# ViTAE-Transformer/SAMRS

Hardware: AMD Instinct MI355X
Metric: images/sec (1024^2, vit_h, 32 boxes/img) SAM box->mask (higher is better)
Workload: dtype f16

## Files before the change

samrs_amd/csrc/encoder_kernels.hip:

```cpp
#include "common.h"
#include "kernels.h"

namespace {

__constant__ float c_mean[3] = {123.675f, 116.28f, 103.53f};
__constant__ float c_std[3] = {58.395f, 57.12f, 57.375f};

template <int PREC>
__global__ void patch_im2col_kernel(const uint8_t* __restrict__ img, uint16_t* __restrict__ A, uint16_t* __restrict__ A_lo,
                                    int n_images, int in_h, int in_w, int grid, int patch) {
    const int P2 = patch * patch;
    const int halves = patch / 8;
    const long total = (long)n_images * grid * grid * patch * halves;
    const long t = (long)blockIdx.x * blockDim.x + threadIdx.x;
    if (t >= total) return;
    const int half = t % halves;
    long u = t / halves;
    const int ky = u % patch; u /= patch;
    const int px = u % grid; u /= grid;
    const int py = u % grid;
    const int im = u / grid;
    const int y = py * patch + ky, x0 = px * patch + half * 8;
    float v[3][8];
#pragma unroll
// ... 421 lines not shown
            const bool real = d0 < HD;
            uint2 o = make_uint2(0u, 0u);
            if (real) {
                o.x = pack2_fast<PREC>(O[dt][4 * g + 0] * inv, O[dt][4 * g + 1] * inv);
                o.y = pack2_fast<PREC>(O[dt][4 * g + 2] * inv, O[dt][4 * g + 3] * inv);
                *reinterpret_cast<uint2*>(orow + d0) = o;
            }
#pragma unroll
            for (int e = 0; e < 4; ++e) {
                const float hv = ET<PREC>::to_float((uint16_t)(((e & 2) ? o.y : o.x) >> (16 * (e & 1))));
                h[4 * g + e] = hv;
                l[4 * g + e] = real ? O[dt][4 * g + e] * inv - hv : 0.f;
                ah = fmaxf(ah, fabsf(hv));
                al = fmaxf(al, fabsf(l[4 * g + e]));
            }
        }
        ah = fmaxf(ah, xhalf_partner(ah));
        al = fmaxf(al, xhalf_partner(al));
        const int bh = mx_scale_byte(ah), bl = mx_scale_byte(al);
        const uint2 ch = make_uint2(fp4_pack8(h, bh), fp4_pack8(h + 8, bh)), cl = make_uint2(fp4_pack8(l, bl), fp4_pack8(l + 8, bl));
        *reinterpret_cast<uint2*>(qh + dt * 16 + 8 * hh) = ch;
        *reinterpret_cast<uint2*>(ql + dt * 16 + 8 * hh) = cl;
        if (hh == 0) {
            const size_t si = mx_scale_index(false, (int)row, head * DT + dt, nst4);
            mx.s_hi[si] = (unsigned char)bh;
            mx.s_lo[si] = (unsigned char)bl;
        }
    }
}

template <int HD>
struct WinCfg {
    static constexpr int WS = 14, N = WS * WS, TK = 2 * WS, NT = N / TK, NP = NT * 32;
    static constexpr int DT = (HD + 31) / 32;
    static constexpr bool ONES = SAMRS_WIN_ONES && DT * 32 > HD;
    __device__ static constexpr int lds_key(int key) { return key + (32 - TK) * (key / TK); }
    static constexpr int VSTR = 228;
    static constexpr int NW = 8, THREADS = NW * 64;
    static constexpr int SSTR = 33;
    static constexpr int K_BYTES = NP * HD * 2;
    static constexpr int VT_BYTES = DT * 32 * VSTR * 2;
    static constexpr int S_BYTES = NW * 32 * SSTR * 4;
    static constexpr int TAB_BYTES = 2 * 32 * HD * 2;
    static constexpr int MAX_D = 1280;
    static constexpr int BIAS_BYTES = 2 * MAX_D * 2;
    static constexpr int LDS_BYTES = K_BYTES + VT_BYTES + S_BYTES + TAB_BYTES + BIAS_BYTES;
};

template <int PREC, int HD, int LO = 0 , int PIPE = 0>
__global__ __launch_bounds__(512) void window_attention_kernel(
    const uint16_t* __restrict__ qkv, const float* __restrict__ qkv_bias, const float* __restrict__ rel_h,
    const float* __restrict__ rel_w, uint16_t* __restrict__ out, int grid, int heads, int n_items,
    uint16_t* __restrict__ out_lo = nullptr , MxOut mx = MxOut(),
    uint32_t lo_heads = 0xffffffffu ) {
    using C = WinCfg<HD>;
    constexpr int KS = HD / 16;
    constexpr bool PL = (PIPE & 1) != 0;
    extern __shared__ __attribute__((aligned(16))) unsigned char smem[];
    uint16_t* Ks = reinterpret_cast<uint16_t*>(smem);
    uint16_t* Vt = reinterpret_cast<uint16_t*>(smem + C::K_BYTES);
    float* Scr = reinterpret_cast<float*>(smem + C::K_BYTES + C::VT_BYTES);
    uint16_t* Tab = reinterpret_cast<uint16_t*>(smem + C::K_BYTES + C::VT_BYTES + C::S_BYTES);
    uint16_t* Bia = Tab + 2 * 32 * HD;

    const int tid = threadIdx.x, lane = tid & 63, wave = tid >> 6;
    const int hh = lane >> 5, ql = lane & 31;
    const int D = heads * HD;
    const int nw = (grid + C::WS - 1) / C::WS;
    const size_t img_rows = (size_t)grid * grid;

    for (int i = tid; i < 2 * 32 * HD; i += C::THREADS) {
        const int t = i / (32 * HD), r = (i / HD) % 32, d = i % HD;
        const float v = r < 2 * C::WS - 1 ? (t ? rel_w : rel_h)[r * HD + d] : 0.f;
        Tab[i] = ET<PREC>::from_float(v);
    }
    for (int i = tid; i < 2 * D; i += C::THREADS) Bia[i] = ET<PREC>::from_float(qkv_bias[D + i]);
    for (int i = tid; i < C::NT * (32 - C::TK) * HD; i += C::THREADS)
        Ks[((i / HD) / (32 - C::TK) * 32 + C::TK + (i / HD) % (32 - C::TK)) * HD + i % HD] = 0;
    for (int i = tid; i < C::DT * 32 * C::VSTR / 2; i += C::THREADS) reinterpret_cast<uint32_t*>(Vt)[i] = 0u;
    if (C::ONES) {
        __syncthreads();
        for (int i = tid; i < C::NP; i += C::THREADS) Vt[HD * C::VSTR + i] = ET<PREC>::from_float(1.0f);
    }

    constexpr int CH = HD / 8;
    constexpr int NKC = C::N * CH, NVI = (C::N / 2) * CH;
    constexpr int PK = (NKC + C::THREADS - 1) / C::THREADS, PV = (NVI + C::THREADS - 1) / C::THREADS;
    const int q = 32 * (wave < C::NT ? wave : 0) + ql;
    const int qc = q < C::N ? q : C::N - 1;
    const int qh = qc / C::WS, qw = qc % C::WS;

    uint4 qf[KS], qfn[PL ? 1 : KS], kreg[PK], v0reg[PV], v1reg[PV];
    auto& qdst = *[&]() { if constexpr (PL) return &qf; else return &qfn; }();
    int n_qoff = -1;
    uint32_t n_pad = 0;
    int n_im = 0, n_head = 0;
#define WIN_TOK(r_, off_, pad_)                                                                                      \
    const int ty_##off_ = y0_ + (r_) / C::WS, tx_##off_ = x0_ + (r_) % C::WS;                                        \
    const bool pad_ = ty_##off_ >= grid || tx_##off_ >= grid;                                                        \
    const int off_ = (min(ty_##off_, grid - 1) * grid + min(tx_##off_, grid - 1)) * (3 * D)
    const uint16_t* n_base = qkv;
    int n_y0 = 0, n_x0 = 0;
#define WIN_HEAD(it_)                                                                                                \
    do {                                                                                                             \
        const int wi_ = (it_) / heads;                                                                               \
        n_head = (it_) % heads;                                                                                      \
        const int win_ = wi_ % (nw * nw);                                                                            \
        n_im = wi_ / (nw * nw);                                                                                      \
        n_y0 = (win_ / nw) * C::WS;                                                                                  \
        n_x0 = (win_ % nw) * C::WS;                                                                                  \
        n_base = qkv + (size_t)n_im * img_rows * (3 * D) + n_head * HD;                                              \
        n_pad = 0u;                                                                                                  \
    } while (0)
#define WIN_LOAD_Q()                                                                                                 \
    do {                                                                                                             \
        const int y0_ = n_y0, x0_ = n_x0;                                                                            \
        WIN_TOK(qc, qo_, qp_);                                                                                       \
        n_qoff = (q < C::N && !qp_) ? qo_ : -1;                                                                      \
        _Pragma("unroll") for (int ks_ = 0; ks_ < KS; ++ks_)                                                         \
            qdst[ks_] = *reinterpret_cast<const uint4*>(n_base + qo_ + 16 * ks_ + 8 * hh);                           \
    } while (0)
    auto slot_field = [](int r, int ch) -> uint32_t { return (uint32_t)(r / C::WS) | ((uint32_t)(r % C::WS) << 4) | ((uint32_t)ch << 8); };
    uint32_t kpk[(PK + 1) / 2], vpk[(PV + 1) / 2];
#pragma unroll
    for (int i = 0; i < (PK + 1) / 2; ++i) kpk[i] = 0u;
#pragma unroll
    for (int i = 0; i < (PV + 1) / 2; ++i) vpk[i] = 0u;
#pragma unroll
    for (int i = 0; i < PK; ++i) {
        const int c = tid + i * C::THREADS;
        if (c < NKC) kpk[i >> 1] |= slot_field(c / CH, c % CH) << (12 * (i & 1));
    }
#pragma unroll
    for (int i = 0; i < PV; ++i) {
        const int c = tid + i * C::THREADS;
        if (c < NVI) vpk[i >> 1] |= slot_field(2 * (c % (C::N / 2)), c / (C::N / 2)) << (12 * (i & 1));
    }
#define WIN_TOK2(dy_, dx_, off_, pad_)                                                                               \
    const int ty_##off_ = y0_ + (dy_), tx_##off_ = x0_ + (dx_);                                                      \
    const bool pad_ = ty_##off_ >= grid || tx_##off_ >= grid;                                                        \
    const int off_ = (min(ty_##off_, grid - 1) * grid + min(tx_##off_, grid - 1)) * (3 * D)
#define WIN_LOAD_K(i_)                                                                                               \
    do {                                                                                                             \
        const int y0_ = n_y0, x0_ = n_x0;                                                                            \
        if (tid + (i_) * C::THREADS < NKC) {                                                                         \
            uint32_t f_ = kpk[(i_) >> 1];                                                                            \
            asm volatile("" : "+v"(f_));           \
            f_ >>= 12 * ((i_) & 1);                                                                                  \
            WIN_TOK2((int)(f_ & 15u), (int)((f_ >> 4) & 15u), ko_, kp_);                                             \
            n_pad |= (uint32_t)kp_ << (i_);                                                                          \
            kreg[i_] = *reinterpret_cast<const uint4*>(n_base + ko_ + D + (int)((f_ >> 8) & 15u) * 8);               \
        }                                                                                                            \
    } while (0)
#define WIN_LOAD_V(i_)                                                                                               \
    do {                                                                                                             \
        const int y0_ = n_y0, x0_ = n_x0;                                                                            \
        if (tid + (i_) * C::THREADS < NVI) {                                                                         \
            uint32_t f_ = vpk[(i_) >> 1];                                                                            \
            asm volatile("" : "+v"(f_));                                                                             \
            f_ >>= 12 * ((i_) & 1);                                                                                  \
            const int dy_ = (int)(f_ & 15u), dx_ = (int)((f_ >> 4) & 15u), ch_ = (int)((f_ >> 8) & 15u);             \
            WIN_TOK2(dy_, dx_, vo0_, vp0_);                                                                          \
            WIN_TOK2(dy_, dx_ + 1, vo1_, vp1_);          \
            n_pad |= ((uint32_t)vp0_ | ((uint32_t)vp1_ << 1)) << (PK + 2 * (i_));                                   \
            v0reg[i_] = *reinterpret_cast<const uint4*>(n_base + vo0_ + 2 * D + ch_ * 8);                            \
            v1reg[i_] = *reinterpret_cast<const uint4*>(n_base + vo1_ + 2 * D + ch_ * 8);                            \
        }                                                                                                            \
    } while (0)
    constexpr int NGK = (PK + 1) / 2, NGRP = 1 + NGK + PV;
    static_assert(NGRP <= C::NT, "issue groups are spread over the key tiles");
#define WIN_GROUP(g_)                                                                                                \
    do {                                                                                                             \
        if ((g_) == 0) { if constexpr (!PL) WIN_LOAD_Q(); }                                                        \
        else if ((g_) <= NGK) {                                                                                      \
            WIN_LOAD_K(2 * ((g_) - 1));                                                                              \
            if (2 * ((g_) - 1) + 1 < PK) WIN_LOAD_K(2 * ((g_) - 1) + 1 < PK ? 2 * ((g_) - 1) + 1 : 0);               \
        } else WIN_LOAD_V((g_) - 1 - NGK < PV ? (g_) - 1 - NGK : 0);                                                 \
    } while (0)
#define WIN_ISSUE(it_)                                                                                               \
    do {                                                                                                             \
        WIN_HEAD(it_);                                                                                               \
        _Pragma("unroll") for (int g_ = 0; g_ < NGRP; ++g_) WIN_GROUP(g_);                                           \
        if constexpr (PL) WIN_LOAD_Q();                                                                              \
    } while (0)

    __syncthreads();
    if constexpr ((PIPE & 2) != 0) {
        if (__builtin_amdgcn_readfirstlane(threadIdx.x) >= 256) __builtin_amdgcn_s_setprio(1);
    }
    int it = blockIdx.x;
#ifdef WIN_TIMING
    unsigned long long wph[6] = {0, 0, 0, 0, 0, 0}, wprev = __builtin_amdgcn_s_memtime();
    const unsigned long long wstart = wprev;
    int n_done = 0;
#define WIN_STAMP(i_) { const unsigned long long tn_ = __builtin_amdgcn_s_memtime(); wph[i_] += tn_ - wprev; wprev = tn_; }
#else
#define WIN_STAMP(i_)
#endif
    if (it < n_items) WIN_ISSUE(it);
    for (; it < n_items; it += gridDim.x) {
        __syncthreads();
        WIN_STAMP(0)
        if (__any(n_pad != 0u)) {
#pragma unroll
            for (int i = 0; i < PK; ++i) {
                const uint4 kb = *reinterpret_cast<const uint4*>(Bia + n_head * HD + ((tid + i * C::THREADS) % CH) * 8);
                kreg[i] = sel4((n_pad >> i) & 1u, kb, kreg[i]);
            }
#pragma unroll
            for (int i = 0; i < PV; ++i) {
                const uint4 vb = *reinterpret_cast<const uint4*>(Bia + D + n_head * HD + ((tid + i * C::THREADS) / (C::N / 2)) % CH * 8);
                v0reg[i] = sel4((n_pad >> (PK + 2 * i)) & 1u, vb, v0reg[i]);
                v1reg[i] = sel4((n_pad >> (PK + 2 * i + 1)) & 1u, vb, v1reg[i]);
            }
        }
#pragma unroll
        for (int i = 0; i < PK; ++i) {
            const int c = tid + i * C::THREADS;
            if (c < NKC) *reinterpret_cast<uint4*>(Ks + C::lds_key(c / CH) * HD + (c % CH) * 8) = kreg[i];
        }
#pragma unroll
        for (int i = 0; i < PV; ++i) {
            const int c = tid + i * C::THREADS;
            if (c < NVI) {
                const int kp = c % (C::N / 2), ch = c / (C::N / 2);
#pragma unroll
                for (int e = 0; e < 8; ++e)
                    *reinterpret_cast<uint32_t*>(Vt + (ch * 8 + e) * C::VSTR + C::lds_key(2 * kp)) = pair_elem(v0reg[i], v1reg[i], e);
            }
        }
        if constexpr (!PL) {
#pragma unroll
            for (int ks = 0; ks < KS; ++ks) qf[ks] = qfn[ks];
        }
        const int qoff = n_qoff;
        const bool qin = qoff >= 0;
        const int im = n_im, head = n_head;
        WIN_STAMP(1)
        __syncthreads();
        WIN_STAMP(2)
        const bool has_next = it + (int)gridDim.x < n_items;
        if (has_next) {
            if (wave >= C::NT) WIN_ISSUE(it + (int)gridDim.x);
            else WIN_HEAD(it + (int)gridDim.x);
        }
        WIN_STAMP(3)
#ifdef WIN_TIMING
        ++n_done;
#endif
        if (wave >= C::NT) continue;

        float* scr = Scr + wave * 32 * C::SSTR + ql * C::SSTR;
        float RH[PL ? 1 : C::WS], BW[16];
        float* rhs = scr;
        {
            const f32x16_t th = tile_times_qT<PREC, HD>(Tab, lane, qf);
            if constexpr (PL) {
                const f32x16_t tw = tile_times_qT<PREC, HD>(Tab + 32 * HD, lane, qf);
#pragma unroll
                for (int r = 0; r < 16; ++r) scr[acc_row(r, hh)] = tw[r];
                wave_lds_sync();
#pragma unroll
                for (int r = 0; r < 16; ++r) {
                    const int c = acc_row(r, hh);
                    BW[r] = c < C::TK ? scr[qw - c % C::WS + C::WS - 1] * LOG2E_F : -INFINITY;
                }
                wave_lds_sync();
#pragma unroll
                for (int r = 0; r < 16; ++r) scr[acc_row(r, hh)] = th[r] * LOG2E_F;
                wave_lds_sync();
                RH[0] = 0.f;
            } else {
#pragma unroll
            for (int r = 0; r < 16; ++r) scr[acc_row(r, hh)] = th[r];
            wave_lds_sync();
#pragma unroll
            for (int j = 0; j < C::WS; ++j) RH[j] = scr[qh - j + C::WS - 1] * LOG2E_F;
            wave_lds_sync();
            const f32x16_t tw = tile_times_qT<PREC, HD>(Tab + 32 * HD, lane, qf);
#pragma unroll
            for (int r = 0; r < 16; ++r) scr[acc_row(r, hh)] = tw[r];
            wave_lds_sync();
#pragma unroll
            for (int r = 0; r < 16; ++r) {
                const int c = acc_row(r, hh);
                BW[r] = c < C::TK ? scr[qw - c % C::WS + C::WS - 1] * LOG2E_F : -INFINITY;
            }
            }
        }

        const float c2 = rsqrtf((float)HD) * LOG2E_F;
        f32x16_t O[C::DT];
#pragma unroll
        for (int dt = 0; dt < C::DT; ++dt)
#pragma unroll
            for (int r = 0; r < 16; ++r) O[dt][r] = 0.f;
        float m_run = -INFINITY, l_run = 0.f;
#ifdef WIN_TIMING
        asm volatile("" :: "v"(RH[0]), "v"(BW[15]));
#endif
        WIN_STAMP(4)

        f32x16_t Sn;
// ... 58 lines not shown
            }
        }
        if constexpr (C::ONES) l_run = ones_row_sum<HD, C::DT>(O, hh);
        else l_run += xhalf_partner(l_run);

#ifdef WIN_TIMING
        asm volatile("" :: "v"(O[0][0]), "v"(O[C::DT - 1][15]), "v"(l_run), "v"(qin), "v"(im), "v"(head));
        WIN_STAMP(5)
        continue;
#endif
        if (qin) {
            const float inv = 1.0f / l_run;
            const size_t orow_i = (size_t)im * img_rows + (size_t)(qoff / (3 * D));
            const size_t obase = orow_i * D + head * HD;
            uint16_t* orow = out + obase;
            if constexpr (LO == 2) store_attention_row_mx<PREC, HD, C::DT>(O, inv, orow, hh, mx, orow_i, head, heads);
            else
#pragma unroll
            for (int dt = 0; dt < C::DT; ++dt)
#pragma unroll
                for (int g = 0; g < 4; ++g) {
                    const int d0 = 32 * dt + 8 * g + 4 * hh;
                    if (d0 < HD) {
                        uint2 o;
                        o.x = pack2_fast<PREC>(O[dt][4 * g + 0] * inv, O[dt][4 * g + 1] * inv);
                        o.y = pack2_fast<PREC>(O[dt][4 * g + 2] * inv, O[dt][4 * g + 3] * inv);
                        *reinterpret_cast<uint2*>(orow + d0) = o;
                        if constexpr (LO == 1) {
                            if ((lo_heads >> (head & 31)) & 1u) {
                                uint2 h, l;
                                split2_pack<PREC>(O[dt][4 * g + 0] * inv, O[dt][4 * g + 1] * inv, h.x, l.x);
                                split2_pack<PREC>(O[dt][4 * g + 2] * inv, O[dt][4 * g + 3] * inv, h.y, l.y);
                                *reinterpret_cast<uint2*>(out_lo + obase + d0) = l;
                            }
                        }
                    }
                }
        }
    }
#ifdef WIN_TIMING
    if (lane == 0) {
        unsigned long long* tp = reinterpret_cast<unsigned long long*>(out) + ((size_t)blockIdx.x * 8 + wave) * 8;
        for (int i = 0; i < 6; ++i) tp[i] = wph[i];
        tp[6] = __builtin_amdgcn_s_memtime() - wstart;
        tp[7] = n_done;
    }
#endif
#undef WIN_ISSUE
#undef WIN_GROUP
#undef WIN_LOAD_V
#undef WIN_LOAD_K
#undef WIN_LOAD_Q
#undef WIN_HEAD
#undef WIN_TOK
#undef WIN_TOK2
}

__device__ __forceinline__ void glds16_sbase(uint32_t voff, const void* sbase, uint32_t m0v) {
    uint32_t keep;
    asm volatile(
        "s_mov_b32 %0, m0\n\t"
        "s_mov_b32 m0, %3\n\t"
        "s_nop 0\n\t"
        "global_load_lds_dwordx4 %1, %2\n\t"
        "s_mov_b32 m0, %0"
        : "=&s"(keep)
        : "v"(voff), "s"(sbase), "s"(m0v)
        : "memory");
}

template <int HD>
__global__ __launch_bounds__(256) void vt_pack_kernel(const uint16_t* __restrict__ qkv, uint16_t* __restrict__ vt, int heads,
                                                      int ntok) {
    __shared__ uint16_t tile[64][HD + 2];
    const int tiles = ntok / 64;
    const int t = blockIdx.x % tiles, P = blockIdx.x / tiles;
    const int head = P % heads, im = P / heads;
    const int D = heads * HD;
    const uint16_t* src = qkv + ((size_t)im * ntok + (size_t)t * 64) * (3 * D) + 2 * D + head * HD;
    constexpr int CH = HD / 8;
    for (int c = threadIdx.x; c < 64 * CH; c += 256) {
        const int r = c / CH, ch = c % CH;
        const uint4 v = *reinterpret_cast<const uint4*>(src + (size_t)r * (3 * D) + ch * 8);
        uint32_t* p = reinterpret_cast<uint32_t*>(&tile[r][ch * 8]);
        p[0] = v.x; p[1] = v.y; p[2] = v.z; p[3] = v.w;
    }
    __syncthreads();
    uint16_t* dst = vt + (size_t)P * HD * ntok + (size_t)t * 64;
    for (int c = threadIdx.x; c < HD * 8; c += 256) {
        const int d = c / 8, c8 = c % 8, k0 = 16 * (c8 >> 1) + 4 * (c8 & 1);
        uint4 o;
        o.x = tile[k0 + 0][d] | ((uint32_t)tile[k0 + 1][d] << 16);
        o.y = tile[k0 + 2][d] | ((uint32_t)tile[k0 + 3][d] << 16);
        o.z = tile[k0 + 8][d] | ((uint32_t)tile[k0 + 9][d] << 16);
        o.w = tile[k0 + 10][d] | ((uint32_t)tile[k0 + 11][d] << 16);
        *reinterpret_cast<uint4*>(dst + (size_t)d * ntok + c8 * 8) = o;
    }
}

template <int HD, int NW = 4>
struct GlbCfg {
    static constexpr int G = 64, KT = 64;
    static constexpr int DT = (HD + 31) / 32;
    static constexpr int VSTR = KT + 8;
    static constexpr int KSTR = HD + 8;
    static constexpr int K_BYTES = KT * KSTR * 2;
    static constexpr int VT_BYTES = DT * 32 * VSTR * 2;
// ... 506 lines not shown
        mean += d * (1.0f / (g + 1));
        m2 += gq + d * d * (160.0f * g / (g + 1));
    }
    const float rstd = 1.0f / sqrtf(m2 * (1.0f / 1280.0f) + eps);
    rowstat[row] = make_float2(rstd, -rstd * mean);
}

hipError_t launch_ln_rowstat(const float* stats, float* rowstat, int rows, float eps, hipStream_t s) {
    if (rows < 1 || !stats || !rowstat) return hipErrorInvalidValue;
    ln_rowstat_kernel<<<(rows + 255) / 256, 256, 0, s>>>(reinterpret_cast<const float4*>(stats), reinterpret_cast<float2*>(rowstat), rows, eps);
    return hipGetLastError();
}

hipError_t launch_rowstats_convert(int prec, const float* X, void* Xh, float* stats, int rows, int D, hipStream_t s) {
    if (D != 1280 || rows < 1) return hipErrorInvalidValue;
    const int blocks = (rows + 3) / 4;
    if (prec == PREC_BF16) rowstats_convert_kernel<PREC_BF16><<<blocks, 256, 0, s>>>(X, (uint16_t*)Xh, reinterpret_cast<float2*>(stats), rows);
    else rowstats_convert_kernel<PREC_F16><<<blocks, 256, 0, s>>>(X, (uint16_t*)Xh, reinterpret_cast<float2*>(stats), rows);
    return hipGetLastError();
}

hipError_t launch_layernorm(int prec, const float* X, const float* gamma, const float* beta, float eps,
                            void* out_et, float* out_f32, int rows_out, int D, int window_mode, int grid,
                            int window, hipStream_t s, void* out_lo, void* mx_q_hi, void* mx_q_lo, void* mx_s_hi, void* mx_s_lo, int ld_out,
                            const int* oc_idx, int n_oc) {
    if (D % 4 || D > LN_MAXV * 256) return hipErrorInvalidValue;
    if (ld_out == 0) ld_out = D;
    if (ld_out < D || ld_out % 4 || (ld_out != D && out_lo)) return hipErrorInvalidValue;
    if (n_oc < 0 || n_oc > 32 || (n_oc && (!oc_idx || !out_et || window_mode || ld_out < D + 64))) return hipErrorInvalidValue;
    MxOut mx;
    if (mx_q_hi) {
        if (!mx_q_lo || !mx_s_hi || !mx_s_lo || !out_et || window_mode || D % MXK) return hipErrorInvalidValue;
        mx.q_hi = (unsigned char*)mx_q_hi; mx.q_lo = (unsigned char*)mx_q_lo; mx.s_hi = (unsigned char*)mx_s_hi; mx.s_lo = (unsigned char*)mx_s_lo;
    }
    const int blocks = (rows_out + 3) / 4;
    if (prec == PREC_BF16)
        layernorm_kernel<PREC_BF16><<<blocks, 256, 0, s>>>(X, gamma, beta, eps, (uint16_t*)out_et, out_f32, rows_out, D, window_mode, grid, window, (uint16_t*)out_lo, mx, ld_out, oc_idx, n_oc);
    else
        layernorm_kernel<PREC_F16><<<blocks, 256, 0, s>>>(X, gamma, beta, eps, (uint16_t*)out_et, out_f32, rows_out, D, window_mode, grid, window, (uint16_t*)out_lo, mx, ld_out, oc_idx, n_oc);
    return hipGetLastError();
}

template <int PREC, int HD, int LO = 0>
static hipError_t launch_win(const void* qkv, const float* qb, const float* rh, const float* rw, void* out, int n_images,
                             int grid, int heads, hipStream_t s, void* out_lo = nullptr, MxOut mx = MxOut(), uint32_t lo_heads = 0xffffffffu) {
    using C = WinCfg<HD>;
#ifdef SAMRS_EXPERIMENTS
    static const int pipe = [] { const char* v = getenv("SAMRS_WIN_PIPE"); return v ? atoi(v) & 3 : 0; }();
    auto k = pipe == 3 ? window_attention_kernel<PREC, HD, LO, 3> : pipe == 2 ? window_attention_kernel<PREC, HD, LO, 2>
           : pipe == 1 ? window_attention_kernel<PREC, HD, LO, 1> : window_attention_kernel<PREC, HD, LO, 0>;
#else
    auto k = window_attention_kernel<PREC, HD, LO, 0>;
#endif
    HIP_CHECK_RET(set_lds(k, C::LDS_BYTES));
    if (heads * HD > C::MAX_D) return hipErrorInvalidValue;
    const int nw = (grid + C::WS - 1) / C::WS;
    const int n_items = n_images * nw * nw * heads;
    static const int n_cu = [] {
        int dev = 0, n = 256;
        if (hipGetDevice(&dev) == hipSuccess) (void)hipDeviceGetAttribute(&n, hipDeviceAttributeMultiprocessorCount, dev);
        return n > 0 ? n : 256;
    }();
    dim3 g(n_items < n_cu ? n_items : n_cu), b(C::THREADS);
    k<<<g, b, C::LDS_BYTES, s>>>((const uint16_t*)qkv, qb, rh, rw, (uint16_t*)out, grid, heads, n_items, (uint16_t*)out_lo, mx, lo_heads);
    return hipGetLastError();
}

hipError_t launch_window_attention(int prec, const void* qkv, const float* qkv_bias, const float* rel_h, const float* rel_w, void* out,
                                   int n_images, int grid, int window, int heads, int head_dim, hipStream_t s, void* out_lo,
                                   void* mx_q_hi, void* mx_q_lo, void* mx_s_hi, void* mx_s_lo, uint32_t lo_heads) {
    if (window != 14) return hipErrorInvalidValue;
    if (heads > 32) lo_heads = 0xffffffffu;
    MxOut mx;
    if (mx_q_hi) {
        if (!mx_q_lo || !mx_s_hi || !mx_s_lo || (heads * ((head_dim + 31) / 32) * 32) % MXK) return hipErrorInvalidValue;
        mx.q_hi = (unsigned char*)mx_q_hi; mx.q_lo = (unsigned char*)mx_q_lo; mx.s_hi = (unsigned char*)mx_s_hi; mx.s_lo = (unsigned char*)mx_s_lo;
    }
#define WIN_CALL(P, H)                                                                                                          \
    return mx_q_hi ? launch_win<P, H, 2>(qkv, qkv_bias, rel_h, rel_w, out, n_images, grid, heads, s, nullptr, mx)               \
         : out_lo ? launch_win<P, H, 1>(qkv, qkv_bias, rel_h, rel_w, out, n_images, grid, heads, s, out_lo, MxOut(), lo_heads)  \
                  : launch_win<P, H, 0>(qkv, qkv_bias, rel_h, rel_w, out, n_images, grid, heads, s)
    if (prec == PREC_BF16) {
        if (head_dim == 64) WIN_CALL(PREC_BF16, 64);
        if (head_dim == 80) WIN_CALL(PREC_BF16, 80);
    } else if (prec == PREC_F16) {
        if (head_dim == 64) WIN_CALL(PREC_F16, 64);
        if (head_dim == 80) WIN_CALL(PREC_F16, 80);
    }
#undef WIN_CALL
    return hipErrorInvalidValue;
}

static int g_glb_waves = [] { const char* v = getenv("SAMRS_GLB_WAVES"); return (v && atoi(v) == 4) ? 4 : 8; }();

template <int PREC, int HD, int NW, int LO = 0>
static hipError_t launch_glb_nw(const void* qkv, const float* rh, const float* rw, void* out, int n_images,
                                int heads, void* vt_ws, hipStream_t s, void* out_lo = nullptr, MxOut mx = MxOut()) {
    using C = GlbCfg<HD, NW>;
    constexpr int NTOK = C::G * C::G;
#ifdef SAMRS_EXPERIMENTS
    static const bool pipe = [] { const char* v = getenv("SAMRS_GLB_PIPE"); return v ? atoi(v) != 0 : false; }();
    auto k = pipe ? global_attention_kernel<PREC, HD, NW, LO, 1> : global_attention_kernel<PREC, HD, NW, LO, 0>;
#else
    auto k = global_attention_kernel<PREC, HD, NW, LO, 0>;
#endif
    HIP_CHECK_RET(set_lds(k, C::LDS_BYTES));
    dim3 g((NTOK / (32 * NW)) * heads * n_images), b(64 * NW);
    k<<<g, b, C::LDS_BYTES, s>>>((const uint16_t*)qkv, (const uint16_t*)vt_ws, rh, rw, (uint16_t*)out, heads, (uint16_t*)out_lo, mx);
    return hipGetLastError();
}

template <int PREC, int HD>
static hipError_t launch_glb(const void* qkv, const float* rh, const float* rw, void* out, int n_images,
                             int heads, void* vt_ws, hipStream_t s, void* out_lo, MxOut mx) {
    constexpr int NTOK = GlbCfg<HD>::G * GlbCfg<HD>::G;
    vt_pack_kernel<HD><<<n_images * heads * (NTOK / 64), 256, 0, s>>>((const uint16_t*)qkv, (uint16_t*)vt_ws, heads, NTOK);
    HIP_CHECK_RET(hipGetLastError());
// ... 59 lines not shown
```

samrs_amd/csrc/upscaler_fused.hip:

```cpp
#include "common.h"
#include "kernels.h"

namespace {

constexpr int UF_THREADS = 512;
constexpr int UF_ROWS = 16;

struct UFArgs {
    const uint16_t *keys, *keys_lo;
    const uint16_t *w1, *w1_lo;
    const float* b1;
    const float* ln;
    const uint16_t *w2, *w2_lo;
    const float* b2;
    const float* hyper;
    float* low;
    int tokens, grid, n_mask_tokens, sel0, n_tiles;
};

template <int PREC, int NSEL, bool SPLIT>
__global__ __launch_bounds__(UF_THREADS) void upscaler_fused_kernel(UFArgs a) {
    extern __shared__ __attribute__((aligned(16))) unsigned char uf_lds[];
    unsigned char* At = uf_lds;
    uint4* W2f = reinterpret_cast<uint4*>(uf_lds + 16384);
    float* Part = reinterpret_cast<float*>(uf_lds + 16384 + 32768);
    float* Out = Part + 4 * 2 * 16 * 64;
    float* cst = Out + 3 * 4 * 64;
    const int tid = threadIdx.x, lane = tid & 63;
    const int wave = __builtin_amdgcn_readfirstlane(tid >> 6);
    const int s1 = wave >> 1, p = wave & 1;
    const int fr = lane & 15, fq = lane >> 4;

    uint4 wf1[4][4], wl1[SPLIT ? 4 : 1][4];
#pragma unroll
    for (int i = 0; i < 4; ++i)
#pragma unroll
        for (int ks = 0; ks < 4; ++ks) {
            const size_t o = (size_t)(s1 * 64 + i * 16 + fr) * 256 + (4 * p + ks) * 32 + fq * 8;
            wf1[i][ks] = *reinterpret_cast<const uint4*>(a.w1 + o);
            if constexpr (SPLIT) wl1[i][ks] = *reinterpret_cast<const uint4*>(a.w1_lo + o);
        }
    for (int idx = tid; idx < 8 * 2 * 64; idx += UF_THREADS) {
        const int i2 = idx >> 7, ks2 = (idx >> 6) & 1, l = idx & 63, r_ = l & 15, q_ = l >> 4;
        const size_t o0 = (size_t)(i2 * 16 + r_) * 64 + 16 * (2 * ks2) + 4 * q_, o1 = o0 + 16;
        const uint2 x0 = *reinterpret_cast<const uint2*>(a.w2 + o0), x1 = *reinterpret_cast<const uint2*>(a.w2 + o1);
        W2f[idx] = make_uint4(x0.x, x0.y, x1.x, x1.y);
        if constexpr (SPLIT) {
            const uint2 y0 = *reinterpret_cast<const uint2*>(a.w2_lo + o0), y1 = *reinterpret_cast<const uint2*>(a.w2_lo + o1);
            W2f[8 * 2 * 64 + idx] = make_uint4(y0.x, y0.y, y1.x, y1.y);
        }
    }
    for (int i = tid; i < 512; i += UF_THREADS)
        cst[i] = i < 256 ? a.b1[i] : (i < 384 ? a.ln[i - 256] : a.b2[i - 384]);

    const int tiles_per_prompt = a.tokens / UF_ROWS;
    const int S = 4 * a.grid;
    const int prow = tid >> 5, pch = tid & 31;
    int tile = blockIdx.x;
    uint4 nh = make_uint4(0u, 0u, 0u, 0u), nl = nh;
    if (tile < a.n_tiles) {
        const size_t o = ((size_t)tile * UF_ROWS + prow) * 256 + pch * 8;
        nh = *reinterpret_cast<const uint4*>(a.keys + o);
        if constexpr (SPLIT) nl = *reinterpret_cast<const uint4*>(a.keys_lo + o);
    }
    for (; tile < a.n_tiles; tile += gridDim.x) {
        const int b = tile / tiles_per_prompt, t0 = (tile - b * tiles_per_prompt) * UF_ROWS;
        *reinterpret_cast<uint4*>(At + ((prow * 32 + (pch ^ prow)) << 4)) = nh;
        if constexpr (SPLIT) *reinterpret_cast<uint4*>(At + 8192 + ((prow * 32 + (pch ^ prow)) << 4)) = nl;
        __syncthreads();
        {
            const int nt = tile + (int)gridDim.x;
            if (nt < a.n_tiles) {
                const size_t o = ((size_t)nt * UF_ROWS + prow) * 256 + pch * 8;
                nh = *reinterpret_cast<const uint4*>(a.keys + o);
                if constexpr (SPLIT) nl = *reinterpret_cast<const uint4*>(a.keys_lo + o);
            }
        }
        float hy[NSEL][8];
#pragma unroll
        for (int c = 0; c < NSEL; ++c) {
            const float* h = a.hyper + ((size_t)b * a.n_mask_tokens + a.sel0 + c) * 32;
#pragma unroll
            for (int half = 0; half < 2; ++half) {
                const float4 t = *reinterpret_cast<const float4*>(h + half * 16 + 4 * fq);
                hy[c][half * 4 + 0] = t.x; hy[c][half * 4 + 1] = t.y; hy[c][half * 4 + 2] = t.z; hy[c][half * 4 + 3] = t.w;
            }
        }
        f32x4_t acc[4];
#pragma unroll
        for (int i = 0; i < 4; ++i) acc[i] = f32x4_t{0.f, 0.f, 0.f, 0.f};
#pragma unroll
        for (int ks = 0; ks < 4; ++ks) {
            const int pos = (fr * 32 + (((4 * p + ks) * 4 + fq) ^ fr)) << 4;
            const uint4 af = *reinterpret_cast<const uint4*>(At + pos);
            if constexpr (SPLIT) {
                const uint4 al = *reinterpret_cast<const uint4*>(At + 8192 + pos);
#pragma unroll
                for (int i = 0; i < 4; ++i) acc[i] = ET<PREC>::mfma16(wf1[i][ks], al, acc[i]);
#pragma unroll
                for (int i = 0; i < 4; ++i) acc[i] = ET<PREC>::mfma16(wl1[i][ks], af, acc[i]);
            }
#pragma unroll
            for (int i = 0; i < 4; ++i) acc[i] = ET<PREC>::mfma16(wf1[i][ks], af, acc[i]);
        }
        float* mine = Part + ((s1 * 2 + p) * 16) * 64 + lane;
#pragma unroll
        for (int i = 0; i < 4; ++i)
#pragma unroll
            for (int r = 0; r < 4; ++r) mine[(i * 4 + r) * 64] = acc[i][r];
        __syncthreads();
        float v[4][4];
        float s = 0.f;
        {
            const float* p0 = Part + ((s1 * 2 + 0) * 16) * 64 + lane;
            const float* p1 = Part + ((s1 * 2 + 1) * 16) * 64 + lane;
#pragma unroll
            for (int i = 0; i < 4; ++i) {
                const float4 bb = *reinterpret_cast<const float4*>(cst + s1 * 64 + i * 16 + 4 * fq);
                const float bv[4] = {bb.x, bb.y, bb.z, bb.w};
#pragma unroll
                for (int r = 0; r < 4; ++r) {
                    v[i][r] = (p0[(i * 4 + r) * 64] + p1[(i * 4 + r) * 64]) + bv[r];
                    s += v[i][r];
                }
            }
        }
        s += __shfl_xor(s, 16, 64);
        s += __shfl_xor(s, 32, 64);
        const float mean = s * (1.0f / 64.0f);
        float q = 0.f;
#pragma unroll
        for (int i = 0; i < 4; ++i)
#pragma unroll
            for (int r = 0; r < 4; ++r) { v[i][r] -= mean; q += v[i][r] * v[i][r]; }
        q += __shfl_xor(q, 16, 64);
        q += __shfl_xor(q, 32, 64);
        const float rstd = 1.0f / sqrtf(q * (1.0f / 64.0f) + 1e-6f);
        uint4 bh[2], bl[2];
#pragma unroll
        for (int ks2 = 0; ks2 < 2; ++ks2) {
            uint32_t hh[4], ll[4];
#pragma unroll
            for (int k = 0; k < 2; ++k) {
                const int i = 2 * ks2 + k;
                const float4 gm = *reinterpret_cast<const float4*>(cst + 256 + i * 16 + 4 * fq);
                const float4 bt = *reinterpret_cast<const float4*>(cst + 320 + i * 16 + 4 * fq);
                const float2_t g01 = gelu_erf2(float2_t{v[i][0] * rstd * gm.x + bt.x, v[i][1] * rstd * gm.y + bt.y});
                const float2_t g23 = gelu_erf2(float2_t{v[i][2] * rstd * gm.z + bt.z, v[i][3] * rstd * gm.w + bt.w});
                split2_pack<PREC>(g01.x, g01.y, hh[2 * k], ll[2 * k]);
                split2_pack<PREC>(g23.x, g23.y, hh[2 * k + 1], ll[2 * k + 1]);
            }
            bh[ks2] = make_uint4(hh[0], hh[1], hh[2], hh[3]);
            bl[ks2] = make_uint4(ll[0], ll[1], ll[2], ll[3]);
        }
        float part[NSEL][2];
#pragma unroll
        for (int c = 0; c < NSEL; ++c) part[c][0] = part[c][1] = 0.f;
#pragma unroll
        for (int il = 0; il < 4; ++il) {
            const int i2 = 4 * p + il;
            f32x4_t d = {0.f, 0.f, 0.f, 0.f};
            const uint4 w0 = W2f[(i2 * 2 + 0) * 64 + lane], w1 = W2f[(i2 * 2 + 1) * 64 + lane];
            if constexpr (SPLIT) {
                const uint4 x0 = W2f[8 * 2 * 64 + (i2 * 2 + 0) * 64 + lane], x1 = W2f[8 * 2 * 64 + (i2 * 2 + 1) * 64 + lane];
                d = ET<PREC>::mfma16(w0, bl[0], d);
                d = ET<PREC>::mfma16(w1, bl[1], d);
                d = ET<PREC>::mfma16(x0, bh[0], d);
                d = ET<PREC>::mfma16(x1, bh[1], d);
            }
            d = ET<PREC>::mfma16(w0, bh[0], d);
            d = ET<PREC>::mfma16(w1, bh[1], d);
            const float4 bb = *reinterpret_cast<const float4*>(cst + 384 + i2 * 16 + 4 * fq);
            const float2_t g01 = gelu_erf2(float2_t{d[0] + bb.x, d[1] + bb.y});
            const float2_t g23 = gelu_erf2(float2_t{d[2] + bb.z, d[3] + bb.w});
#pragma unroll
            for (int c = 0; c < NSEL; ++c) {
                const float* h = hy[c] + (il & 1) * 4;
                part[c][il >> 1] += h[0] * g01.x + h[1] * g01.y + h[2] * g23.x + h[3] * g23.y;
            }
        }
#pragma unroll
        for (int c = 0; c < NSEL; ++c)
#pragma unroll
            for (int sl = 0; sl < 2; ++sl) {
                float x = part[c][sl];
                x += __shfl_xor(x, 16, 64);
                x += __shfl_xor(x, 32, 64);
                if (fq == sl) {
                    const int s2 = 2 * p + sl;
                    Out[(c * 4 + 2 * (s1 >> 1) + (s2 >> 1)) * 64 + 4 * fr + 2 * (s1 & 1) + (s2 & 1)] = x;
                }
            }
        __syncthreads();
        for (int idx = tid; idx < NSEL * 256; idx += UF_THREADS) {
            const int c = idx >> 8, yl = (idx >> 6) & 3, xl = idx & 63;
            const int y = t0 / a.grid, x0 = t0 - y * a.grid;
            a.low[(((size_t)b * NSEL + c) * S + 4 * y + yl) * S + 4 * x0 + xl] = Out[(c * 4 + yl) * 64 + xl];
        }
    }
}

constexpr int UF_LDS = 16384 + 32768 + 32768 + 3 * 4 * 64 * 4 + 512 * 4;

}

hipError_t launch_upscaler_fused(int prec, const void* keys, const void* keys_lo, const void* w1, const void* w1_lo, const float* b1,
                                 const float* ln, const void* w2, const void* w2_lo, const float* b2, const float* hyper, float* low,
                                 int n, int grid, int n_mask_tokens, int sel0, int n_sel, hipStream_t s) {
    const bool split = keys_lo && w1_lo && w2_lo;
    if ((keys_lo || w1_lo || w2_lo) && !split) return hipErrorInvalidValue;
    if (n < 1 || grid % UF_ROWS || (n_sel != 1 && n_sel != 3)) return hipErrorInvalidValue;
    static const int n_cu = [] {
        int dev = 0, c = 256;
        if (hipGetDevice(&dev) == hipSuccess) (void)hipDeviceGetAttribute(&c, hipDeviceAttributeMultiprocessorCount, dev);
        return c > 0 ? c : 256;
    }();
    UFArgs a;
    a.keys = (const uint16_t*)keys; a.keys_lo = (const uint16_t*)keys_lo;
    a.w1 = (const uint16_t*)w1; a.w1_lo = (const uint16_t*)w1_lo; a.b1 = b1; a.ln = ln;
    a.w2 = (const uint16_t*)w2; a.w2_lo = (const uint16_t*)w2_lo; a.b2 = b2; a.hyper = hyper; a.low = low;
    a.tokens = grid * grid; a.grid = grid; a.n_mask_tokens = n_mask_tokens; a.sel0 = sel0;
    a.n_tiles = n * (a.tokens / UF_ROWS);
    const int blocks = a.n_tiles < n_cu ? a.n_tiles : n_cu;
#define UF_LAUNCH(P, NS, SP)                                                                                                 \
    do {                                                                                                                     \
        auto k = upscaler_fused_kernel<P, NS, SP>;                                                                           \
        HIP_CHECK_RET(hipFuncSetAttribute(reinterpret_cast<const void*>(k), hipFuncAttributeMaxDynamicSharedMemorySize, UF_LDS)); \
        k<<<blocks, UF_THREADS, UF_LDS, s>>>(a);                                                                             \
    } while (0)
#define UF_SEL(P, SP) do { if (n_sel == 1) UF_LAUNCH(P, 1, SP); else UF_LAUNCH(P, 3, SP); } while (0)
    if (prec == PREC_BF16) { if (split) UF_SEL(PREC_BF16, true); else UF_SEL(PREC_BF16, false); }
    else if (prec == PREC_F16) { if (split) UF_SEL(PREC_F16, true); else UF_SEL(PREC_F16, false); }
    else return hipErrorInvalidValue;
#undef UF_SEL
#undef UF_LAUNCH
    return hipGetLastError();
}
```

Before: 147.5.

## Skip padded query strips in window attention; widen upscaler tile to two groups

The window attention kernel now computes the real query count of each edge window and lets waves whose 32-query strip is entirely padding skip the attention math, with a fast reciprocal-multiply replacing the division for row/column. Separately, the fused upscaler processes two 16-token groups per tile, which halves tile-loop iterations and reuses the register-resident weights across more rows at the cost of roughly doubled LDS. Both paths are on by default and can be switched off through environment variables.

```diff
diff --git a/samrs_amd/csrc/encoder_kernels.hip b/samrs_amd/csrc/encoder_kernels.hip
--- a/samrs_amd/csrc/encoder_kernels.hip
+++ b/samrs_amd/csrc/encoder_kernels.hip
@@ -497,7 +497,8 @@
     const uint16_t* __restrict__ qkv, const float* __restrict__ qkv_bias, const float* __restrict__ rel_h,
     const float* __restrict__ rel_w, uint16_t* __restrict__ out, int grid, int heads, int n_items,
     uint16_t* __restrict__ out_lo = nullptr , MxOut mx = MxOut(),
-    uint32_t lo_heads = 0xffffffffu ) {
+    uint32_t lo_heads = 0xffffffffu ,
+    int dense = 1 ) {
     using C = WinCfg<HD>;
     constexpr int KS = HD / 16;
     constexpr bool PL = (PIPE & 1) != 0;
@@ -509,6 +510,7 @@
     uint16_t* Bia = Tab + 2 * 32 * HD;
 
     const int tid = threadIdx.x, lane = tid & 63, wave = tid >> 6;
+    const int wave_u = __builtin_amdgcn_readfirstlane(wave);
     const int hh = lane >> 5, ql = lane & 31;
     const int D = heads * HD;
     const int nw = (grid + C::WS - 1) / C::WS;
@@ -532,20 +534,20 @@
     constexpr int NKC = C::N * CH, NVI = (C::N / 2) * CH;
     constexpr int PK = (NKC + C::THREADS - 1) / C::THREADS, PV = (NVI + C::THREADS - 1) / C::THREADS;
     const int q = 32 * (wave < C::NT ? wave : 0) + ql;
-    const int qc = q < C::N ? q : C::N - 1;
-    const int qh = qc / C::WS, qw = qc % C::WS;
+    auto slot_row = [](int q_, int vw_) -> int { return (int)(((uint32_t)q_ * ((65536u + (uint32_t)vw_ - 1u) / (uint32_t)vw_)) >> 16); };
 
     uint4 qf[KS], qfn[PL ? 1 : KS], kreg[PK], v0reg[PV], v1reg[PV];
     auto& qdst = *[&]() { if constexpr (PL) return &qf; else return &qfn; }();
     int n_qoff = -1;
     uint32_t n_pad = 0;
     int n_im = 0, n_head = 0;
-#define WIN_TOK(r_, off_, pad_)                                                                                      \
-    const int ty_##off_ = y0_ + (r_) / C::WS, tx_##off_ = x0_ + (r_) % C::WS;                                        \
+#define WIN_TOK2(dy_, dx_, off_, pad_)                                                                               \
+    const int ty_##off_ = y0_ + (dy_), tx_##off_ = x0_ + (dx_);                                                      \
     const bool pad_ = ty_##off_ >= grid || tx_##off_ >= grid;                                                        \
     const int off_ = (min(ty_##off_, grid - 1) * grid + min(tx_##off_, grid - 1)) * (3 * D)
     const uint16_t* n_base = qkv;
     int n_y0 = 0, n_x0 = 0;
+    int n_vw = C::WS, n_nq = C::N;
 #define WIN_HEAD(it_)                                                                                                \
     do {                                                                                                             \
         const int wi_ = (it_) / heads;                                                                               \
@@ -556,12 +558,15 @@
         n_x0 = (win_ % nw) * C::WS;                                                                                  \
         n_base = qkv + (size_t)n_im * img_rows * (3 * D) + n_head * HD;                                              \
         n_pad = 0u;                                                                                                  \
+        n_vw = dense ? min(C::WS, grid - n_x0) : C::WS;                                                              \
+        n_nq = dense ? min(C::WS, grid - n_y0) * n_vw : C::N;                                                        \
     } while (0)
 #define WIN_LOAD_Q()                                                                                                 \
     do {                                                                                                             \
         const int y0_ = n_y0, x0_ = n_x0;                                                                            \
-        WIN_TOK(qc, qo_, qp_);                                                                                       \
-        n_qoff = (q < C::N && !qp_) ? qo_ : -1;                                                                      \
+        const int qc_ = min(q, n_nq - 1), qh_ = slot_row(qc_, n_vw);                                                 \
+        WIN_TOK2(qh_, qc_ - qh_ * n_vw, qo_, qp_);                                                                   \
+        n_qoff = (q < n_nq && !qp_) ? qo_ : -1;                                                                      \
         _Pragma("unroll") for (int ks_ = 0; ks_ < KS; ++ks_)                                                         \
             qdst[ks_] = *reinterpret_cast<const uint4*>(n_base + qo_ + 16 * ks_ + 8 * hh);                           \
     } while (0)
@@ -581,10 +586,6 @@
         const int c = tid + i * C::THREADS;
         if (c < NVI) vpk[i >> 1] |= slot_field(2 * (c % (C::N / 2)), c / (C::N / 2)) << (12 * (i & 1));
     }
-#define WIN_TOK2(dy_, dx_, off_, pad_)                                                                               \
-    const int ty_##off_ = y0_ + (dy_), tx_##off_ = x0_ + (dx_);                                                      \
-    const bool pad_ = ty_##off_ >= grid || tx_##off_ >= grid;                                                        \
-    const int off_ = (min(ty_##off_, grid - 1) * grid + min(tx_##off_, grid - 1)) * (3 * D)
 #define WIN_LOAD_K(i_)                                                                                               \
     do {                                                                                                             \
         const int y0_ = n_y0, x0_ = n_x0;                                                                            \
@@ -681,19 +682,21 @@
         const int qoff = n_qoff;
         const bool qin = qoff >= 0;
         const int im = n_im, head = n_head;
+        const int n_strips = (n_nq + 31) >> 5;
+        const int qc = min(q, n_nq - 1), qh = slot_row(qc, n_vw), qw = qc - qh * n_vw;
         WIN_STAMP(1)
         __syncthreads();
         WIN_STAMP(2)
         const bool has_next = it + (int)gridDim.x < n_items;
         if (has_next) {
-            if (wave >= C::NT) WIN_ISSUE(it + (int)gridDim.x);
+            if (wave_u >= n_strips) WIN_ISSUE(it + (int)gridDim.x);
             else WIN_HEAD(it + (int)gridDim.x);
         }
         WIN_STAMP(3)
 #ifdef WIN_TIMING
         ++n_done;
 #endif
-        if (wave >= C::NT) continue;
+        if (wave_u >= n_strips) continue;
 
         float* scr = Scr + wave * 32 * C::SSTR + ql * C::SSTR;
         float RH[PL ? 1 : C::WS], BW[16];
@@ -858,7 +861,6 @@
 #undef WIN_LOAD_K
 #undef WIN_LOAD_Q
 #undef WIN_HEAD
-#undef WIN_TOK
 #undef WIN_TOK2
 }
 
@@ -1471,6 +1473,7 @@
 #else
     auto k = window_attention_kernel<PREC, HD, LO, 0>;
 #endif
+    static const int dense = [] { const char* v = getenv("SAMRS_WIN_DENSE"); return (v && atoi(v) == 0) ? 0 : 1; }();
     HIP_CHECK_RET(set_lds(k, C::LDS_BYTES));
     if (heads * HD > C::MAX_D) return hipErrorInvalidValue;
     const int nw = (grid + C::WS - 1) / C::WS;
@@ -1481,7 +1484,8 @@
         return n > 0 ? n : 256;
     }();
     dim3 g(n_items < n_cu ? n_items : n_cu), b(C::THREADS);
-    k<<<g, b, C::LDS_BYTES, s>>>((const uint16_t*)qkv, qb, rh, rw, (uint16_t*)out, grid, heads, n_items, (uint16_t*)out_lo, mx, lo_heads);
+    k<<<g, b, C::LDS_BYTES, s>>>((const uint16_t*)qkv, qb, rh, rw, (uint16_t*)out, grid, heads, n_items, (uint16_t*)out_lo, mx, lo_heads,
+                                 dense);
     return hipGetLastError();
 }
 
diff --git a/samrs_amd/csrc/upscaler_fused.hip b/samrs_amd/csrc/upscaler_fused.hip
--- a/samrs_amd/csrc/upscaler_fused.hip
+++ b/samrs_amd/csrc/upscaler_fused.hip
@@ -1,10 +1,12 @@
+#include <cstdlib>
+
 #include "common.h"
 #include "kernels.h"
 
 namespace {
 
 constexpr int UF_THREADS = 512;
-constexpr int UF_ROWS = 16;
+constexpr int UF_GROUP = 16;
 
 struct UFArgs {
     const uint16_t *keys, *keys_lo;
@@ -18,14 +20,16 @@
     int tokens, grid, n_mask_tokens, sel0, n_tiles;
 };
 
-template <int PREC, int NSEL, bool SPLIT>
+template <int PREC, int NSEL, bool SPLIT, int NH >
 __global__ __launch_bounds__(UF_THREADS) void upscaler_fused_kernel(UFArgs a) {
     extern __shared__ __attribute__((aligned(16))) unsigned char uf_lds[];
+    constexpr int ROWS = NH * UF_GROUP;
+    constexpr int AT_LO = ROWS * 512;
     unsigned char* At = uf_lds;
-    uint4* W2f = reinterpret_cast<uint4*>(uf_lds + 16384);
-    float* Part = reinterpret_cast<float*>(uf_lds + 16384 + 32768);
-    float* Out = Part + 4 * 2 * 16 * 64;
-    float* cst = Out + 3 * 4 * 64;
+    uint4* W2f = reinterpret_cast<uint4*>(uf_lds + 2 * AT_LO);
+    float* Part = reinterpret_cast<float*>(uf_lds + 2 * AT_LO + 32768);
+    float* Out = Part + 4 * 2 * NH * 16 * 64;
+    float* cst = Out + 3 * NH * 4 * 64;
     const int tid = threadIdx.x, lane = tid & 63;
     const int wave = __builtin_amdgcn_readfirstlane(tid >> 6);
     const int s1 = wave >> 1, p = wave & 1;
@@ -53,27 +57,39 @@
     for (int i = tid; i < 512; i += UF_THREADS)
         cst[i] = i < 256 ? a.b1[i] : (i < 384 ? a.ln[i - 256] : a.b2[i - 384]);
 
-    const int tiles_per_prompt = a.tokens / UF_ROWS;
+    const int tiles_per_prompt = a.tokens / ROWS;
     const int S = 4 * a.grid;
     const int prow = tid >> 5, pch = tid & 31;
     int tile = blockIdx.x;
-    uint4 nh = make_uint4(0u, 0u, 0u, 0u), nl = nh;
+    uint4 nh[NH], nl[NH];
+#pragma unroll
+    for (int h = 0; h < NH; ++h) nh[h] = nl[h] = make_uint4(0u, 0u, 0u, 0u);
     if (tile < a.n_tiles) {
-        const size_t o = ((size_t)tile * UF_ROWS + prow) * 256 + pch * 8;
-        nh = *reinterpret_cast<const uint4*>(a.keys + o);
-        if constexpr (SPLIT) nl = *reinterpret_cast<const uint4*>(a.keys_lo + o);
+#pragma unroll
+        for (int h = 0; h < NH; ++h) {
+            const size_t o = ((size_t)tile * ROWS + h * UF_GROUP + prow) * 256 + pch * 8;
+            nh[h] = *reinterpret_cast<const uint4*>(a.keys + o);
+            if constexpr (SPLIT) nl[h] = *reinterpret_cast<const uint4*>(a.keys_lo + o);
+        }
     }
     for (; tile < a.n_tiles; tile += gridDim.x) {
-        const int b = tile / tiles_per_prompt, t0 = (tile - b * tiles_per_prompt) * UF_ROWS;
-        *reinterpret_cast<uint4*>(At + ((prow * 32 + (pch ^ prow)) << 4)) = nh;
-        if constexpr (SPLIT) *reinterpret_cast<uint4*>(At + 8192 + ((prow * 32 + (pch ^ prow)) << 4)) = nl;
+        const int b = tile / tiles_per_prompt, t0 = (tile - b * tiles_per_prompt) * ROWS;
+#pragma unroll
+        for (int h = 0; h < NH; ++h) {
+            const int pos = (((h * UF_GROUP + prow) * 32 + (pch ^ prow)) << 4);
+            *reinterpret_cast<uint4*>(At + pos) = nh[h];
+            if constexpr (SPLIT) *reinterpret_cast<uint4*>(At + AT_LO + pos) = nl[h];
+        }
         __syncthreads();
         {
             const int nt = tile + (int)gridDim.x;
             if (nt < a.n_tiles) {
-                const size_t o = ((size_t)nt * UF_ROWS + prow) * 256 + pch * 8;
-                nh = *reinterpret_cast<const uint4*>(a.keys + o);
-                if constexpr (SPLIT) nl = *reinterpret_cast<const uint4*>(a.keys_lo + o);
+#pragma unroll
+                for (int h = 0; h < NH; ++h) {
+                    const size_t o = ((size_t)nt * ROWS + h * UF_GROUP + prow) * 256 + pch * 8;
+                    nh[h] = *reinterpret_cast<const uint4*>(a.keys + o);
+                    if constexpr (SPLIT) nl[h] = *reinterpret_cast<const uint4*>(a.keys_lo + o);
+                }
             }
         }
         float hy[NSEL][8];
@@ -86,34 +102,38 @@
                 hy[c][half * 4 + 0] = t.x; hy[c][half * 4 + 1] = t.y; hy[c][half * 4 + 2] = t.z; hy[c][half * 4 + 3] = t.w;
             }
         }
-        f32x4_t acc[4];
-#pragma unroll
-        for (int i = 0; i < 4; ++i) acc[i] = f32x4_t{0.f, 0.f, 0.f, 0.f};
-#pragma unroll
-        for (int ks = 0; ks < 4; ++ks) {
-            const int pos = (fr * 32 + (((4 * p + ks) * 4 + fq) ^ fr)) << 4;
-            const uint4 af = *reinterpret_cast<const uint4*>(At + pos);
-            if constexpr (SPLIT) {
-                const uint4 al = *reinterpret_cast<const uint4*>(At + 8192 + pos);
-#pragma unroll
-                for (int i = 0; i < 4; ++i) acc[i] = ET<PREC>::mfma16(wf1[i][ks], al, acc[i]);
-#pragma unroll
-                for (int i = 0; i < 4; ++i) acc[i] = ET<PREC>::mfma16(wl1[i][ks], af, acc[i]);
-            }
-#pragma unroll
-            for (int i = 0; i < 4; ++i) acc[i] = ET<PREC>::mfma16(wf1[i][ks], af, acc[i]);
-        }
-        float* mine = Part + ((s1 * 2 + p) * 16) * 64 + lane;
-#pragma unroll
-        for (int i = 0; i < 4; ++i)
-#pragma unroll
-            for (int r = 0; r < 4; ++r) mine[(i * 4 + r) * 64] = acc[i][r];
+#pragma unroll
+        for (int h = 0; h < NH; ++h) {
+            f32x4_t acc[4];
+#pragma unroll
+            for (int i = 0; i < 4; ++i) acc[i] = f32x4_t{0.f, 0.f, 0.f, 0.f};
+#pragma unroll
+            for (int ks = 0; ks < 4; ++ks) {
+                const int pos = ((h * UF_GROUP + fr) * 32 + (((4 * p + ks) * 4 + fq) ^ fr)) << 4;
+                const uint4 af = *reinterpret_cast<const uint4*>(At + pos);
+                if constexpr (SPLIT) {
+                    const uint4 al = *reinterpret_cast<const uint4*>(At + AT_LO + pos);
+#pragma unroll
+                    for (int i = 0; i < 4; ++i) acc[i] = ET<PREC>::mfma16(wf1[i][ks], al, acc[i]);
+#pragma unroll
+                    for (int i = 0; i < 4; ++i) acc[i] = ET<PREC>::mfma16(wl1[i][ks], af, acc[i]);
+                }
+#pragma unroll
+                for (int i = 0; i < 4; ++i) acc[i] = ET<PREC>::mfma16(wf1[i][ks], af, acc[i]);
+            }
+            float* mine = Part + (((s1 * 2 + p) * NH + h) * 16) * 64 + lane;
+#pragma unroll
+            for (int i = 0; i < 4; ++i)
+#pragma unroll
+                for (int r = 0; r < 4; ++r) mine[(i * 4 + r) * 64] = acc[i][r];
+        }
         __syncthreads();
+        const int hg = NH == 2 ? p : 0;
         float v[4][4];
         float s = 0.f;
         {
-            const float* p0 = Part + ((s1 * 2 + 0) * 16) * 64 + lane;
-            const float* p1 = Part + ((s1 * 2 + 1) * 16) * 64 + lane;
+            const float* p0 = Part + (((s1 * 2 + 0) * NH + hg) * 16) * 64 + lane;
+            const float* p1 = Part + (((s1 * 2 + 1) * NH + hg) * 16) * 64 + lane;
 #pragma unroll
             for (int i = 0; i < 4; ++i) {
                 const float4 bb = *reinterpret_cast<const float4*>(cst + s1 * 64 + i * 16 + 4 * fq);
@@ -153,12 +173,16 @@
             bh[ks2] = make_uint4(hh[0], hh[1], hh[2], hh[3]);
             bl[ks2] = make_uint4(ll[0], ll[1], ll[2], ll[3]);
         }
-        float part[NSEL][2];
-#pragma unroll
-        for (int c = 0; c < NSEL; ++c) part[c][0] = part[c][1] = 0.f;
-#pragma unroll
-        for (int il = 0; il < 4; ++il) {
-            const int i2 = 4 * p + il;
+        constexpr int NS2 = 2 * NH;
+        const int s2_0 = NH == 2 ? 0 : 2 * p;
+        float part[NSEL];
+#pragma unroll
+        for (int il = 0; il < 2 * NS2; ++il) {
+            if ((il & 1) == 0) {
+#pragma unroll
+                for (int c = 0; c < NSEL; ++c) part[c] = 0.f;
+            }
+            const int i2 = 2 * s2_0 + il;
             f32x4_t d = {0.f, 0.f, 0.f, 0.f};
             const uint4 w0 = W2f[(i2 * 2 + 0) * 64 + lane], w1 = W2f[(i2 * 2 + 1) * 64 + lane];
             if constexpr (SPLIT) {
@@ -176,31 +200,30 @@
 #pragma unroll
             for (int c = 0; c < NSEL; ++c) {
                 const float* h = hy[c] + (il & 1) * 4;
-                part[c][il >> 1] += h[0] * g01.x + h[1] * g01.y + h[2] * g23.x + h[3] * g23.y;
-            }
-        }
-#pragma unroll
-        for (int c = 0; c < NSEL; ++c)
-#pragma unroll
-            for (int sl = 0; sl < 2; ++sl) {
-                float x = part[c][sl];
-                x += __shfl_xor(x, 16, 64);
-                x += __shfl_xor(x, 32, 64);
-                if (fq == sl) {
-                    const int s2 = 2 * p + sl;
-                    Out[(c * 4 + 2 * (s1 >> 1) + (s2 >> 1)) * 64 + 4 * fr + 2 * (s1 & 1) + (s2 & 1)] = x;
-                }
-            }
+                part[c] += h[0] * g01.x + h[1] * g01.y + h[2] * g23.x + h[3] * g23.y;
+            }
+            if (il & 1) {
+                const int sl = il >> 1, s2 = s2_0 + sl;
+#pragma unroll
+                for (int c = 0; c < NSEL; ++c) {
+                    float x = part[c];
+                    x += __shfl_xor(x, 16, 64);
+                    x += __shfl_xor(x, 32, 64);
+                    if (fq == sl) Out[((c * NH + hg) * 4 + 2 * (s1 >> 1) + (s2 >> 1)) * 64 + 4 * fr + 2 * (s1 & 1) + (s2 & 1)] = x;
+                }
+            }
+        }
         __syncthreads();
-        for (int idx = tid; idx < NSEL * 256; idx += UF_THREADS) {
-            const int c = idx >> 8, yl = (idx >> 6) & 3, xl = idx & 63;
-            const int y = t0 / a.grid, x0 = t0 - y * a.grid;
-            a.low[(((size_t)b * NSEL + c) * S + 4 * y + yl) * S + 4 * x0 + xl] = Out[(c * 4 + yl) * 64 + xl];
+        for (int idx = tid; idx < NSEL * NH * 256; idx += UF_THREADS) {
+            const int ch = idx >> 8, c = ch / NH, tg = t0 + (ch % NH) * UF_GROUP, yl = (idx >> 6) & 3, xl = idx & 63;
+            const int y = tg / a.grid, x0 = tg - y * a.grid;
+            a.low[(((size_t)b * NSEL + c) * S + 4 * y + yl) * S + 4 * x0 + xl] = Out[(ch * 4 + yl) * 64 + xl];
         }
     }
 }
 
-constexpr int UF_LDS = 16384 + 32768 + 32768 + 3 * 4 * 64 * 4 + 512 * 4;
+constexpr int uf_lds_bytes(int nh) { return nh * 16384 + 32768 + nh * 32768 + 3 * nh * 4 * 64 * 4 + 512 * 4; }
+static_assert(uf_lds_bytes(2) <= 160 * 1024, "the 32-token tile must fit the CU's LDS");
 
 }
 
@@ -209,7 +232,8 @@
                                  int n, int grid, int n_mask_tokens, int sel0, int n_sel, hipStream_t s) {
     const bool split = keys_lo && w1_lo && w2_lo;
     if ((keys_lo || w1_lo || w2_lo) && !split) return hipErrorInvalidValue;
-    if (n < 1 || grid % UF_ROWS || (n_sel != 1 && n_sel != 3)) return hipErrorInvalidValue;
+    if (n < 1 || grid % UF_GROUP || (n_sel != 1 && n_sel != 3)) return hipErrorInvalidValue;
+    static const int n_groups = [] { const char* v = getenv("SAMRS_UPSCALER_TILE"); return (v && atoi(v) == 16) ? 1 : 2; }();
     static const int n_cu = [] {
         int dev = 0, c = 256;
         if (hipGetDevice(&dev) == hipSuccess) (void)hipDeviceGetAttribute(&c, hipDeviceAttributeMultiprocessorCount, dev);
@@ -220,13 +244,14 @@
     a.w1 = (const uint16_t*)w1; a.w1_lo = (const uint16_t*)w1_lo; a.b1 = b1; a.ln = ln;
     a.w2 = (const uint16_t*)w2; a.w2_lo = (const uint16_t*)w2_lo; a.b2 = b2; a.hyper = hyper; a.low = low;
     a.tokens = grid * grid; a.grid = grid; a.n_mask_tokens = n_mask_tokens; a.sel0 = sel0;
-    a.n_tiles = n * (a.tokens / UF_ROWS);
+    a.n_tiles = n * (a.tokens / (n_groups * UF_GROUP));
     const int blocks = a.n_tiles < n_cu ? a.n_tiles : n_cu;
 #define UF_LAUNCH(P, NS, SP)                                                                                                 \
     do {                                                                                                                     \
-        auto k = upscaler_fused_kernel<P, NS, SP>;                                                                           \
-        HIP_CHECK_RET(hipFuncSetAttribute(reinterpret_cast<const void*>(k), hipFuncAttributeMaxDynamicSharedMemorySize, UF_LDS)); \
-        k<<<blocks, UF_THREADS, UF_LDS, s>>>(a);                                                                             \
+        auto k = n_groups == 2 ? upscaler_fused_kernel<P, NS, SP, 2> : upscaler_fused_kernel<P, NS, SP, 1>;                  \
+        const int lds = uf_lds_bytes(n_groups);                                                                              \
+        HIP_CHECK_RET(hipFuncSetAttribute(reinterpret_cast<const void*>(k), hipFuncAttributeMaxDynamicSharedMemorySize, lds)); \
+        k<<<blocks, UF_THREADS, lds, s>>>(a);                                                                                \
     } while (0)
 #define UF_SEL(P, SP) do { if (n_sel == 1) UF_LAUNCH(P, 1, SP); else UF_LAUNCH(P, 3, SP); } while (0)
     if (prec == PREC_BF16) { if (split) UF_SEL(PREC_BF16, true); else UF_SEL(PREC_BF16, false); }
```

After: 149.3 (median of 6 runs). 1.2% higher.
